# OPENAIRINTERFACE/openairinterface5g

Measured on AMD Instinct MI355X. Metric: ldpc_decoder_coded_throughput, higher is better.
Workload: dtype int8

## Files before the change

### openairinterface5g_amd/csrc/ldpc_dec_fast_core.h

```cpp
#ifndef LDPC_DEC_FAST_CORE_H
#define LDPC_DEC_FAST_CORE_H
#include "ldpc_dec_core.h"

#if !defined(__HIPCC__)
struct uint2 { uint32_t x, y; };
#endif
typedef short ldpc_v2i __attribute__((ext_vector_type(2)));
typedef unsigned short ldpc_v2u __attribute__((ext_vector_type(2)));

#if defined(__HIP_DEVICE_COMPILE__)
LDPC_HD uint32_t ldpc_perm(uint32_t s0, uint32_t s1, uint32_t sel) { return __builtin_amdgcn_perm(s0, s1, sel); }
LDPC_HD uint32_t ldpc_alignbyte(uint32_t hi, uint32_t lo, uint32_t sh) { return __builtin_amdgcn_alignbyte(hi, lo, sh); }
LDPC_HD uint32_t ldpc_umulhi(uint32_t a, uint32_t b) { return __umulhi(a, b); }
#else
LDPC_HD uint32_t ldpc_perm(uint32_t s0, uint32_t s1, uint32_t sel)
{
  const uint64_t src = ((uint64_t)s0 << 32) | s1;
  uint32_t r = 0;
  for (int i = 0; i < 4; i++) {
    const uint32_t s = (sel >> (8 * i)) & 0xff;
    const uint32_t b = s <= 7 ? (uint32_t)((src >> (8 * s)) & 0xff) : (s == 0x0c ? 0u : 0xffu);
    r |= b << (8 * i);
  }
  return r;
}
LDPC_HD uint32_t ldpc_alignbyte(uint32_t hi, uint32_t lo, uint32_t sh)
{
  return (uint32_t)(((((uint64_t)hi) << 32) | lo) >> (8 * (sh & 3)));
}
LDPC_HD uint32_t ldpc_umulhi(uint32_t a, uint32_t b) { return (uint32_t)(((uint64_t)a * b) >> 32); }
#endif

LDPC_HD ldpc_v2i ldpc_as_v2i(uint32_t x) { return __builtin_bit_cast(ldpc_v2i, x); }
LDPC_HD ldpc_v2u ldpc_as_v2u(uint32_t x) { return __builtin_bit_cast(ldpc_v2u, x); }
LDPC_HD uint32_t ldpc_u2u32(ldpc_v2u x) { return __builtin_bit_cast(uint32_t, x); }
LDPC_HD ldpc_v2u ldpc_splatu(unsigned v) { return (ldpc_v2u){(unsigned short)v, (unsigned short)v}; }
LDPC_HD ldpc_v2u ldpc_pminu(ldpc_v2u a, ldpc_v2u b) { return __builtin_elementwise_min(a, b); }
LDPC_HD ldpc_v2u ldpc_pmaxu(ldpc_v2u a, ldpc_v2u b) { return __builtin_elementwise_max(a, b); }
#define LDPC_KEY_NEUTRAL 0xfbffu
LDPC_HD ldpc_v2u ldpc_pmin3_keys(ldpc_v2u a, ldpc_v2u b, ldpc_v2u c)
{
#if defined(__HIP_DEVICE_COMPILE__)
  uint32_t r;
  asm("v_pk_maximum3_f16 %0, %1, %2, %3" : "=v"(r) : "v"(__builtin_bit_cast(uint32_t, a)), "v"(__builtin_bit_cast(uint32_t, b)),
      "v"(__builtin_bit_cast(uint32_t, c)));
  return __builtin_bit_cast(ldpc_v2u, r);
#else
  return __builtin_elementwise_min(__builtin_elementwise_min(a, b), c);
#endif
}
LDPC_HD uint32_t ldpc_as_u32(ldpc_v2i x) { return __builtin_bit_cast(uint32_t, x); }
LDPC_HD ldpc_v2i ldpc_splat(int v) { return (ldpc_v2i){(short)v, (short)v}; }
LDPC_HD ldpc_v2i ldpc_pmin(ldpc_v2i a, ldpc_v2i b) { return __builtin_elementwise_min(a, b); }
LDPC_HD ldpc_v2i ldpc_pmax(ldpc_v2i a, ldpc_v2i b) { return __builtin_elementwise_max(a, b); }
LDPC_HD ldpc_v2i ldpc_unpack_lo(uint32_t w) { return ldpc_as_v2i(ldpc_perm(0u, w, 0x0c010c00u)); }
LDPC_HD ldpc_v2i ldpc_unpack_hi(uint32_t w) { return ldpc_as_v2i(ldpc_perm(0u, w, 0x0c030c02u)); }
LDPC_HD uint32_t ldpc_pack4(ldpc_v2i lo, ldpc_v2i hi) { return ldpc_perm(ldpc_as_u32(hi), ldpc_as_u32(lo), 0x06040200u); }

struct ldpc_fast_lds {
  uint8_t *base;
  uint8_t *r;
  uint8_t *app;
  uint8_t *ext;
  const uint32_t *etbl, *ctbl, *rowtbl, *coltbl;
  const uint8_t *gllr;
  int ext_global;
};

#if defined(__HIP_DEVICE_COMPILE__)
LDPC_HD uint32_t ldpc_lds_addr(const uint8_t *p) { return (uint32_t)(uintptr_t)(const __attribute__((address_space(3))) uint8_t *)p; }
LDPC_HD uint32_t ldpc_lds_ld32(const uint8_t *, uint32_t a) { return *(const __attribute__((address_space(3))) uint32_t *)a; }
#else
LDPC_HD uint32_t ldpc_lds_addr(const uint8_t *) { return 0u; }
LDPC_HD uint32_t ldpc_lds_ld32(const uint8_t *base, uint32_t a) { return *reinterpret_cast<const uint32_t *>(base + a); }
#endif
LDPC_HD uint32_t ldpc_window_al(const uint8_t *base, uint32_t a, uint32_t sh)
{
  return ldpc_alignbyte(ldpc_lds_ld32(base, a + 4u), ldpc_lds_ld32(base, a), sh);
}
LDPC_HD uint32_t ldpc_window(const uint8_t *base, uint32_t off) { return ldpc_window_al(base, off & ~3u, off); }

LDPC_HD uint32_t ldpc_fast_odd_lanes(uint32_t parw, bool ext, uint32_t extl, uint32_t exth, int D)
{
  uint32_t np = parw >> 7;
  if (ext)
    np ^= ldpc_perm(exth, extl, 0x07050301u);
  if (D & 1)
    np = ~np;
  return np & 0x01010101u;
}
LDPC_HD uint32_t ldpc_fast_valid_lanes(int valid) { return valid > 0 ? 0x01010101u : 0u; }

template <bool IS_EXT, bool P1 = false>
LDPC_HD void ldpc_fast_cn_edge(const ldpc_fast_lds &L, uint32_t info, int t, uint32_t rw, bool first, uint32_t &dl, uint32_t &dh,
                               uint32_t &parw, uint32_t &extl, uint32_t &exth)
{
  uint32_t al, ah, rl, rh;
  if (IS_EXT) {
    const uint32_t lw = L.ext_global ? (*reinterpret_cast<const uint32_t *>(L.gllr + info + (uint32_t)t) ^ 0x80808080u)
                                     : ldpc_lds_ld32(L.base, info + (uint32_t)t);
    al = ldpc_perm(0x80808080u, lw, 0x05010400u);
    ah = ldpc_perm(0x80808080u, lw, 0x05030402u);
    if (first) {
      extl = al + (P1 ? 0x00800080u : ldpc_perm(0u, rw, 0x0c010c00u));
      exth = ah + (P1 ? 0x00800080u : ldpc_perm(0u, rw, 0x0c030c02u));
    }
    rl = 0x00800080u;
    rh = 0x00800080u;
  } else {
    const uint32_t aw = ldpc_window(L.base, info + (uint32_t)t);
    if (first)
      parw ^= aw;
    al = ldpc_perm(0x80808080u, aw, 0x05010400u);
    ah = ldpc_perm(0x80808080u, aw, 0x05030402u);
    rl = P1 ? 0x00800080u : ldpc_perm(0u, rw, 0x0c010c00u);
    rh = P1 ? 0x00800080u : ldpc_perm(0u, rw, 0x0c030c02u);
  }
  dl = al - rl;
  dh = ah - rh;
}

template <int D, bool EXT, int MODE, bool P1 = false>
LDPC_HD uint32_t ldpc_fast_cn(const ldpc_fast_lds &L, int e0, int j, int Z, int rstride, int boff_r = 0, int boff_a = 0)
{
  const int t = 4 * j + boff_r, ta = 4 * j + boff_a;
  constexpr bool KEEP = MODE == 0;
  uint32_t d_lo[MODE <= 1 ? D : 1], d_hi[MODE <= 1 ? D : 1], g_lo[KEEP ? D : 1], g_hi[KEEP ? D : 1];
  ldpc_v2u m1l = ldpc_splatu(0xffff), m2l = m1l, m1h = m1l, m2h = m1l;
  uint32_t sxl = 0, sxh = 0, parw = 0, extl = 0, exth = 0;
  uint8_t *rrow = L.r + e0 * rstride + t;
  uint8_t *rpad = rrow + (j == 0 ? Z : 0);
#pragma unroll
  for (int k = 0; k < D; k++) {
    const uint32_t info = L.etbl[e0 + k];
    const uint32_t rw = P1 ? 0u : *reinterpret_cast<const uint32_t *>(rrow + k * rstride);
    uint32_t dl, dh;
    if (EXT && k == D - 1)
      ldpc_fast_cn_edge<true, P1>(L, info, t, rw, true, dl, dh, parw, extl, exth);
    else
      ldpc_fast_cn_edge<false, P1>(L, info, ta, rw, true, dl, dh, parw, extl, exth);
    if (MODE <= 1) {
      d_lo[k] = dl;
      d_hi[k] = dh;
    }
    const ldpc_v2u ml = ldpc_pmaxu(ldpc_as_v2u(dl), ldpc_as_v2u(0x00010000u - dl));
    const ldpc_v2u mh = ldpc_pmaxu(ldpc_as_v2u(dh), ldpc_as_v2u(0x00010000u - dh));
    if (KEEP) {
      g_lo[k] = ldpc_u2u32(ml);
      g_hi[k] = ldpc_u2u32(mh);
    }
    sxl ^= dl;
    sxh ^= dh;
    m2l = ldpc_pminu(m2l, ldpc_pmaxu(m1l, ml));
    m1l = ldpc_pminu(m1l, ml);
    m2h = ldpc_pminu(m2h, ldpc_pmaxu(m1h, mh));
    m1h = ldpc_pminu(m1h, mh);
  }
  const ldpc_v2u cap = ldpc_splatu(0x8000 + 127);
  m1l = ldpc_pminu(m1l, cap); m2l = ldpc_pminu(m2l, cap);
  m1h = ldpc_pminu(m1h, cap); m2h = ldpc_pminu(m2h, cap);
  const uint32_t sl = (ldpc_u2u32(m1l) - 0x80008000u) + ldpc_u2u32(m2l), sh = (ldpc_u2u32(m1h) - 0x80008000u) + ldpc_u2u32(m2h);
  if ((D - 1) & 1) {
    sxl ^= 0x80008000u;
    sxh ^= 0x80008000u;
  }
  const uint32_t sx4 = ldpc_perm(sxh, sxl, 0x07050301u);
#pragma unroll
  for (int k = 0; k < D; k++) {
    uint32_t dl, dh;
    if (MODE <= 1) {
      dl = d_lo[k];
      dh = d_hi[k];
    } else {
      const uint32_t info = L.etbl[e0 + k];
      const uint32_t rw = P1 ? 0u : *reinterpret_cast<const uint32_t *>(rrow + k * rstride);
      if (EXT && k == D - 1)
        ldpc_fast_cn_edge<true, P1>(L, info, t, rw, false, dl, dh, parw, extl, exth);
      else
        ldpc_fast_cn_edge<false, P1>(L, info, ta, rw, false, dl, dh, parw, extl, exth);
    }
    const ldpc_v2u ml = KEEP ? ldpc_as_v2u(g_lo[k]) : ldpc_pmaxu(ldpc_as_v2u(dl), ldpc_as_v2u(0x00010000u - dl));
    const ldpc_v2u mh = KEEP ? ldpc_as_v2u(g_hi[k]) : ldpc_pmaxu(ldpc_as_v2u(dh), ldpc_as_v2u(0x00010000u - dh));
    const uint32_t ol = sl - ldpc_u2u32(ldpc_pminu(ml, m2l)), oh = sh - ldpc_u2u32(ldpc_pminu(mh, m2h));
    const uint32_t o4 = ldpc_perm(oh, ol, 0x06040200u);
    const uint32_t n4 = ((sx4 ^ ldpc_perm(dh, dl, 0x07050301u)) >> 7) & 0x01010101u;
    const uint32_t w = (o4 ^ (0x80808080u - n4)) + n4;
    *reinterpret_cast<uint32_t *>(rrow + k * rstride) = w;
    *reinterpret_cast<uint32_t *>(rpad + k * rstride) = w;
  }
  return ldpc_fast_odd_lanes(parw, EXT, extl, exth, D);
}

template <int D, bool EXT, bool P1 = false>
LDPC_HD uint32_t ldpc_fast_cn_ps(const ldpc_fast_lds &L, int e0, int j, int Z, int rstride, int boff_r = 0, int boff_a = 0)
{
  const int t = 4 * j + boff_r, ta = 4 * j + boff_a;
  constexpr int NP = D / 2;
  uint32_t m_lo[D], m_hi[D], p_lo[NP], p_hi[NP], s4[D];
  const ldpc_v2u cap = ldpc_splatu(0x8000 + 127);
  uint32_t sx4 = 0, parw = 0, extl = 0, exth = 0;
  uint8_t *rrow = L.r + e0 * rstride + t;
  uint8_t *rpad = rrow + (j == 0 ? Z : 0);
#pragma unroll
  for (int k = 0; k < D; k++) {
    const uint32_t info = L.etbl[e0 + k];
    const uint32_t rw = P1 ? 0u : *reinterpret_cast<const uint32_t *>(rrow + k * rstride);
    uint32_t dl, dh;
    if (EXT && k == D - 1)
      ldpc_fast_cn_edge<true, P1>(L, info, t, rw, true, dl, dh, parw, extl, exth);
    else
      ldpc_fast_cn_edge<false, P1>(L, info, ta, rw, true, dl, dh, parw, extl, exth);
    const ldpc_v2u ml = ldpc_pmaxu(ldpc_as_v2u(dl), ldpc_as_v2u(0x00010000u - dl));
    const ldpc_v2u mh = ldpc_pmaxu(ldpc_as_v2u(dh), ldpc_as_v2u(0x00010000u - dh));
    m_lo[k] = ldpc_u2u32(ml);
    m_hi[k] = ldpc_u2u32(mh);
    s4[k] = ldpc_perm(dh, dl, 0x07050301u);
    sx4 ^= s4[k];
    if ((k & 1) && k < D - 1) {
      const int i = k / 2;
      p_lo[i] = ldpc_u2u32(ldpc_pmin3_keys(i ? ldpc_as_v2u(p_lo[i - 1]) : cap, ldpc_as_v2u(m_lo[k - 1]), ml));
      p_hi[i] = ldpc_u2u32(ldpc_pmin3_keys(i ? ldpc_as_v2u(p_hi[i - 1]) : cap, ldpc_as_v2u(m_hi[k - 1]), mh));
    }
  }
  if (!((D - 1) & 1))
    sx4 ^= 0x80808080u;
  auto put = [&](int k, ldpc_v2u ol, ldpc_v2u oh) {
    const uint32_t o4 = ldpc_perm(ldpc_u2u32(oh), ldpc_u2u32(ol), 0x06040200u);
    const uint32_t x4 = sx4 ^ s4[k];
    const uint32_t w = (o4 ^ x4) + (x4 & 0x01010101u);
    *reinterpret_cast<uint32_t *>(rrow + k * rstride) = w;
    *reinterpret_cast<uint32_t *>(rpad + k * rstride) = w;
  };
  ldpc_v2u sl = cap, sh = cap;
  if (D & 1) {
    put(D - 1, ldpc_as_v2u(p_lo[NP - 1]), ldpc_as_v2u(p_hi[NP - 1]));
    sl = ldpc_as_v2u(m_lo[D - 1]);
    sh = ldpc_as_v2u(m_hi[D - 1]);
  }
#pragma unroll
  for (int i = NP - 1; i >= 0; i--) {
    const int k0 = 2 * i, k1 = 2 * i + 1;
    const ldpc_v2u pvl = i ? ldpc_as_v2u(p_lo[i - 1]) : cap, pvh = i ? ldpc_as_v2u(p_hi[i - 1]) : cap;
    const ldpc_v2u a0l = ldpc_as_v2u(m_lo[k0]), a0h = ldpc_as_v2u(m_hi[k0]), a1l = ldpc_as_v2u(m_lo[k1]), a1h = ldpc_as_v2u(m_hi[k1]);
    const bool last = !(D & 1) && i == NP - 1;
    put(k0, last ? ldpc_pminu(pvl, a1l) : ldpc_pmin3_keys(pvl, a1l, sl), last ? ldpc_pminu(pvh, a1h) : ldpc_pmin3_keys(pvh, a1h, sh));
    put(k1, last ? ldpc_pminu(pvl, a0l) : ldpc_pmin3_keys(pvl, a0l, sl), last ? ldpc_pminu(pvh, a0h) : ldpc_pmin3_keys(pvh, a0h, sh));
    if (i > 0) {
      sl = last ? ldpc_pminu(a0l, a1l) : ldpc_pmin3_keys(sl, a0l, a1l);
      sh = last ? ldpc_pminu(a0h, a1h) : ldpc_pmin3_keys(sh, a0h, a1h);
    }
  }
  return ldpc_fast_odd_lanes(parw, EXT, extl, exth, D);
}

template <int D, bool EXT, bool P1 = false>
LDPC_HD uint32_t ldpc_fast_cn_ps2(const ldpc_fast_lds &L, int e0a, int ja, int e0b, int jb, int Z, int rstride, uint32_t &mask_b)
{
  constexpr int N = 2, NP = D / 2;
  const int e0[N] = {e0a, e0b}, t[N] = {4 * ja, 4 * jb};
  uint32_t m_lo[N][D], m_hi[N][D], p_lo[N][NP > 0 ? NP : 1], p_hi[N][NP > 0 ? NP : 1], s4[N][D];
  const ldpc_v2u cap = ldpc_splatu(0x8000 + 127);
  uint32_t sx4[N] = {0, 0}, parw[N] = {0, 0}, extl[N] = {0, 0}, exth[N] = {0, 0};
  uint8_t *rrow[N], *rpad[N];
#pragma unroll
  for (int n = 0; n < N; n++) {
    rrow[n] = L.r + e0[n] * rstride + t[n];
    rpad[n] = rrow[n] + (t[n] == 0 ? Z : 0);
  }
#pragma unroll
  for (int k = 0; k < D; k++) {
    uint32_t info[N], rw[N];
#pragma unroll
    for (int n = 0; n < N; n++) {
      info[n] = L.etbl[e0[n] + k];
      rw[n] = P1 ? 0u : *reinterpret_cast<const uint32_t *>(rrow[n] + k * rstride);
    }
#pragma unroll
    for (int n = 0; n < N; n++) {
      uint32_t dl, dh;
      if (EXT && k == D - 1)
        ldpc_fast_cn_edge<true, P1>(L, info[n], t[n], rw[n], true, dl, dh, parw[n], extl[n], exth[n]);
      else
        ldpc_fast_cn_edge<false, P1>(L, info[n], t[n], rw[n], true, dl, dh, parw[n], extl[n], exth[n]);
      const ldpc_v2u ml = ldpc_pmaxu(ldpc_as_v2u(dl), ldpc_as_v2u(0x00010000u - dl));
      const ldpc_v2u mh = ldpc_pmaxu(ldpc_as_v2u(dh), ldpc_as_v2u(0x00010000u - dh));
      m_lo[n][k] = ldpc_u2u32(ml);
      m_hi[n][k] = ldpc_u2u32(mh);
      s4[n][k] = ldpc_perm(dh, dl, 0x07050301u);
      sx4[n] ^= s4[n][k];
      if ((k & 1) && k < D - 1) {
        const int i = k / 2;
        p_lo[n][i] = ldpc_u2u32(ldpc_pmin3_keys(i ? ldpc_as_v2u(p_lo[n][i - 1]) : cap, ldpc_as_v2u(m_lo[n][k - 1]), ml));
        p_hi[n][i] = ldpc_u2u32(ldpc_pmin3_keys(i ? ldpc_as_v2u(p_hi[n][i - 1]) : cap, ldpc_as_v2u(m_hi[n][k - 1]), mh));
      }
    }
  }
  if (!((D - 1) & 1)) {
    sx4[0] ^= 0x80808080u;
    sx4[1] ^= 0x80808080u;
  }
  auto put = [&](int n, int k, ldpc_v2u ol, ldpc_v2u oh) {
    const uint32_t o4 = ldpc_perm(ldpc_u2u32(oh), ldpc_u2u32(ol), 0x06040200u);
    const uint32_t x4 = sx4[n] ^ s4[n][k];
    const uint32_t w = (o4 ^ x4) + (x4 & 0x01010101u);
    *reinterpret_cast<uint32_t *>(rrow[n] + k * rstride) = w;
    *reinterpret_cast<uint32_t *>(rpad[n] + k * rstride) = w;
  };
  ldpc_v2u sl[N] = {cap, cap}, sh[N] = {cap, cap};
  if (D & 1) {
#pragma unroll
    for (int n = 0; n < N; n++) {
      put(n, D - 1, NP ? ldpc_as_v2u(p_lo[n][NP - 1]) : cap, NP ? ldpc_as_v2u(p_hi[n][NP - 1]) : cap);
      sl[n] = ldpc_as_v2u(m_lo[n][D - 1]);
      sh[n] = ldpc_as_v2u(m_hi[n][D - 1]);
    }
  }
#pragma unroll
  for (int i = NP - 1; i >= 0; i--) {
    const int k0 = 2 * i, k1 = 2 * i + 1;
    const bool last = !(D & 1) && i == NP - 1;
#pragma unroll
    for (int n = 0; n < N; n++) {
      const ldpc_v2u pvl = i ? ldpc_as_v2u(p_lo[n][i - 1]) : cap, pvh = i ? ldpc_as_v2u(p_hi[n][i - 1]) : cap;
      const ldpc_v2u a0l = ldpc_as_v2u(m_lo[n][k0]), a0h = ldpc_as_v2u(m_hi[n][k0]), a1l = ldpc_as_v2u(m_lo[n][k1]), a1h = ldpc_as_v2u(m_hi[n][k1]);
      put(n, k0, last ? ldpc_pminu(pvl, a1l) : ldpc_pmin3_keys(pvl, a1l, sl[n]), last ? ldpc_pminu(pvh, a1h) : ldpc_pmin3_keys(pvh, a1h, sh[n]));
      put(n, k1, last ? ldpc_pminu(pvl, a0l) : ldpc_pmin3_keys(pvl, a0l, sl[n]), last ? ldpc_pminu(pvh, a0h) : ldpc_pmin3_keys(pvh, a0h, sh[n]));
      if (i > 0) {
        sl[n] = last ? ldpc_pminu(a0l, a1l) : ldpc_pmin3_keys(sl[n], a0l, a1l);
        sh[n] = last ? ldpc_pminu(a0h, a1h) : ldpc_pmin3_keys(sh[n], a0h, a1h);
      }
    }
  }
  uint32_t out[N];
#pragma unroll
  for (int n = 0; n < N; n++) {
    out[n] = ldpc_fast_odd_lanes(parw[n], EXT, extl[n], exth[n], D);
  }
  mask_b = out[1];
  return out[0];
}
#if defined(__HIP_DEVICE_COMPILE__) && defined(LDPC_CN2_NOINLINE)
#define LDPC_CN2_ATTR __device__ __attribute__((noinline))
#else
#define LDPC_CN2_ATTR LDPC_HD
#endif
template <bool P1 = false>
LDPC_CN2_ATTR uint32_t ldpc_fast_cn2_dispatch(int deg, const ldpc_fast_lds &L, int e0a, int ja, int e0b, int jb, int Z, int rstride, uint32_t &mask_b)
{
  switch (deg) {
    case 3: return ldpc_fast_cn_ps2<3, true, P1>(L, e0a, ja, e0b, jb, Z, rstride, mask_b);
    case 4: return ldpc_fast_cn_ps2<4, true, P1>(L, e0a, ja, e0b, jb, Z, rstride, mask_b);
    default: return ldpc_fast_cn_ps2<5, true, P1>(L, e0a, ja, e0b, jb, Z, rstride, mask_b);
  }
}

#if defined(__HIP_DEVICE_COMPILE__)
__device__ __forceinline__ uint32_t ldpc_swap_pair(uint32_t v) { return (uint32_t)__builtin_amdgcn_update_dpp(0, (int)v, 0xB1 , 0xf, 0xf, false); }
template <bool P1>
__device__ __forceinline__ uint32_t ldpc_fast_cn19_pair(const ldpc_fast_lds &L, int e0, int j, int Z, int rstride, int half)
{
  constexpr int N = 10, NP = N / 2;
  const int t = 4 * j;
  const int ebase = e0 + (half ? 10 : 0);
  uint32_t m_lo[N], m_hi[N], p_lo[NP], p_hi[NP], s4[N];
  const ldpc_v2u cap = ldpc_splatu(0x8000 + 127);
  uint32_t sx4 = 0, parw = 0, extl = 0, exth = 0;
  uint8_t *rrow = L.r + ebase * rstride + t;
  uint8_t *rpad = rrow + (j == 0 ? Z : 0);
#pragma unroll
  for (int k = 0; k < N; k++) {
    const bool live = k < N - 1 || !half;
    const int kk = live ? k : N - 2;
    const uint32_t info = L.etbl[ebase + kk];
    const uint32_t rw = P1 ? 0u : *reinterpret_cast<const uint32_t *>(rrow + kk * rstride);
    uint32_t dl, dh, pw = 0;
    ldpc_fast_cn_edge<false, P1>(L, info, t, rw, true, dl, dh, pw, extl, exth);
    ldpc_v2u ml = ldpc_pmaxu(ldpc_as_v2u(dl), ldpc_as_v2u(0x00010000u - dl));
    ldpc_v2u mh = ldpc_pmaxu(ldpc_as_v2u(dh), ldpc_as_v2u(0x00010000u - dh));
    uint32_t sg = ldpc_perm(dh, dl, 0x07050301u);
    if (!live) {
      ml = mh = ldpc_splatu(LDPC_KEY_NEUTRAL);
      sg = 0u;
      pw = 0u;
    }
    m_lo[k] = ldpc_u2u32(ml); m_hi[k] = ldpc_u2u32(mh);
    s4[k] = sg;
    sx4 ^= sg;
    parw ^= pw;
    if (k & 1) {
      const int i = k / 2;
      p_lo[i] = ldpc_u2u32(ldpc_pmin3_keys(i ? ldpc_as_v2u(p_lo[i - 1]) : cap, ldpc_as_v2u(m_lo[k - 1]), ml));
      p_hi[i] = ldpc_u2u32(ldpc_pmin3_keys(i ? ldpc_as_v2u(p_hi[i - 1]) : cap, ldpc_as_v2u(m_hi[k - 1]), mh));
    }
  }
  ldpc_v2u sl = ldpc_as_v2u(ldpc_swap_pair(p_lo[NP - 1])), sh = ldpc_as_v2u(ldpc_swap_pair(p_hi[NP - 1]));
  sx4 ^= ldpc_swap_pair(sx4);
  parw ^= ldpc_swap_pair(parw);
  sx4 ^= 0x80808080u;
#pragma unroll
  for (int i = NP - 1; i >= 0; i--) {
    const ldpc_v2u pvl = i ? ldpc_as_v2u(p_lo[i - 1]) : cap, pvh = i ? ldpc_as_v2u(p_hi[i - 1]) : cap;
#pragma unroll
    for (int q = 0; q < 2; q++) {
      const int k = 2 * i + q, ko = 2 * i + 1 - q;
      const bool live = k < N - 1 || !half;
      const ldpc_v2u ol = ldpc_pmin3_keys(pvl, ldpc_as_v2u(m_lo[ko]), sl), oh = ldpc_pmin3_keys(pvh, ldpc_as_v2u(m_hi[ko]), sh);
      const uint32_t o4 = ldpc_perm(ldpc_u2u32(oh), ldpc_u2u32(ol), 0x06040200u);
      const uint32_t x4 = sx4 ^ s4[k];
      const uint32_t w = (o4 ^ x4) + (x4 & 0x01010101u);
      if (live) {
        *reinterpret_cast<uint32_t *>(rrow + k * rstride) = w;
        *reinterpret_cast<uint32_t *>(rpad + k * rstride) = w;
      }
    }
    if (i > 0) {
      sl = ldpc_pmin3_keys(sl, ldpc_as_v2u(m_lo[2 * i]), ldpc_as_v2u(m_lo[2 * i + 1]));
      sh = ldpc_pmin3_keys(sh, ldpc_as_v2u(m_hi[2 * i]), ldpc_as_v2u(m_hi[2 * i + 1]));
    }
  }
  return ldpc_fast_odd_lanes(parw, false, 0u, 0u, 19);
}
#endif

LDPC_HD uint32_t ldpc_fast_pc(const ldpc_fast_lds &L, int D, int ext, int e0, int j, int rstride)
{
  const int t = 4 * j;
  uint32_t parw = 0;
  const int ncore_edges = ext ? D - 1 : D;
  int k = 0;
  for (; k + 4 <= ncore_edges; k += 4) {
    uint32_t info[4], lo[4], hi[4];
#pragma unroll
    for (int i = 0; i < 4; i++)
      info[i] = L.etbl[e0 + k + i] + (uint32_t)t;
#pragma unroll
    for (int i = 0; i < 4; i++) {
      lo[i] = ldpc_lds_ld32(L.base, info[i] & ~3u);
      hi[i] = ldpc_lds_ld32(L.base, (info[i] & ~3u) + 4u);
    }
#pragma unroll
    for (int i = 0; i < 4; i++)
      parw ^= ldpc_alignbyte(hi[i], lo[i], info[i]);
  }
  for (; k < ncore_edges; k++)
    parw ^= ldpc_window(L.base, L.etbl[e0 + k] + (uint32_t)t);
  uint32_t extl = 0, exth = 0;
  if (ext) {
    const uint32_t info = L.etbl[e0 + D - 1];
    const uint32_t lw = L.ext_global ? (*reinterpret_cast<const uint32_t *>(L.gllr + info + (uint32_t)t) ^ 0x80808080u)
                                     : ldpc_lds_ld32(L.base, info + (uint32_t)t);
    const uint32_t rw = *reinterpret_cast<const uint32_t *>(L.r + (e0 + D - 1) * rstride + t);
    extl = ldpc_perm(0x80808080u, lw, 0x05010400u) + ldpc_perm(0u, rw, 0x0c010c00u);
    exth = ldpc_perm(0x80808080u, lw, 0x05030402u) + ldpc_perm(0u, rw, 0x0c030c02u);
  }
  return ldpc_fast_odd_lanes(parw, ext != 0, extl, exth, D);
}

#ifndef LDPC_F_MODE_D19
#define LDPC_F_MODE_D19 2
#endif
template <bool P1 = false>
LDPC_HD uint32_t ldpc_fast_cn_dispatch(int deg, int ext, const ldpc_fast_lds &L, int e0, int j, int Z, int rstride, int boff_r = 0,
                                       int boff_a = 0)
{
  if (!ext) {
    switch (deg) {
      case 19: return ldpc_fast_cn<19, false, LDPC_F_MODE_D19, P1>(L, e0, j, Z, rstride, boff_r, boff_a);
      case 10: return ldpc_fast_cn_ps<10, false, P1>(L, e0, j, Z, rstride, boff_r, boff_a);
      default: return ldpc_fast_cn_ps<8, false, P1>(L, e0, j, Z, rstride, boff_r, boff_a);
    }
  }
  switch (deg) {
    case 3: return ldpc_fast_cn_ps<3, true, P1>(L, e0, j, Z, rstride, boff_r, boff_a);
    case 4: return ldpc_fast_cn_ps<4, true, P1>(L, e0, j, Z, rstride, boff_r, boff_a);
    case 5: return ldpc_fast_cn_ps<5, true, P1>(L, e0, j, Z, rstride, boff_r, boff_a);
    case 6: return ldpc_fast_cn_ps<6, true, P1>(L, e0, j, Z, rstride, boff_r, boff_a);
    case 7: return ldpc_fast_cn_ps<7, true, P1>(L, e0, j, Z, rstride, boff_r, boff_a);
    case 8: return ldpc_fast_cn_ps<8, true, P1>(L, e0, j, Z, rstride, boff_r, boff_a);
    case 9: return ldpc_fast_cn_ps<9, true, P1>(L, e0, j, Z, rstride, boff_r, boff_a);
    default: return ldpc_fast_cn_ps<10, true, P1>(L, e0, j, Z, rstride, boff_r, boff_a);
  }
}

LDPC_HD void ldpc_fast_bn_gather_from(const ldpc_fast_lds &L, int first, int maxdeg, int j, int Z, int boff_r, uint32_t &acc_e,
                                      uint32_t &acc_o)
{
  const int u = 4 * j;
  const uint2 *tbl = reinterpret_cast<const uint2 *>(L.ctbl) + first;
  int k = 0;
  uint2 ce[4];
  if (maxdeg >= 4) {
#pragma unroll
    for (int i = 0; i < 4; i++)
      ce[i] = tbl[i];
  }
  for (; k + 4 <= maxdeg; k += 4) {
    uint32_t lo[4], hi[4], ph[4];
#pragma unroll
    for (int i = 0; i < 4; i++) {
      const uint32_t q = (uint32_t)u + ce[i].x;
      const uint32_t p = q < q - (uint32_t)Z ? q : q - (uint32_t)Z;
      const uint32_t a = ce[i].y + p + (uint32_t)boff_r;
      lo[i] = ldpc_lds_ld32(L.base, a);
      hi[i] = ldpc_lds_ld32(L.base, a + 4u);
      ph[i] = q;
    }
    if (k + 8 <= maxdeg) {
#pragma unroll
      for (int i = 0; i < 4; i++)
        ce[i] = tbl[k + 4 + i];
    }
#pragma unroll
    for (int i = 0; i < 4; i++) {
      const uint32_t w = ldpc_alignbyte(hi[i], lo[i], ph[i]);
      acc_e += w & 0x00ff00ffu;
      acc_o += (w >> 8) & 0x00ff00ffu;
    }
  }
  for (; k < maxdeg; k++) {
    const uint2 c1 = tbl[k];
    const uint32_t q = (uint32_t)u + c1.x;
    const uint32_t p = q < q - (uint32_t)Z ? q : q - (uint32_t)Z;
    const uint32_t v = ldpc_window_al(L.base, c1.y + p + (uint32_t)boff_r, q);
    acc_e += v & 0x00ff00ffu;
    acc_o += (v >> 8) & 0x00ff00ffu;
  }
}
LDPC_HD void ldpc_fast_bn_gather(const ldpc_fast_lds &L, uint32_t colrec, int maxdeg, int j, int Z, int boff_r, uint32_t &acc_e,
                                 uint32_t &acc_o)
{
  ldpc_fast_bn_gather_from(L, (int)(colrec >> 16), maxdeg, j, Z, boff_r, acc_e, acc_o);
}
LDPC_HD void ldpc_fast_bn_finish(const ldpc_fast_lds &L, int c, int deg, int j, int Z, int astride, uint32_t llr_word, uint32_t acc_e,
                                 uint32_t acc_o, int boff_a)
{
  const int u = 4 * j;
  const uint32_t lw = llr_word ^ 0x80808080u;
  acc_e += lw & 0x00ff00ffu;
  acc_o += (lw >> 8) & 0x00ff00ffu;
#if defined(__HIP_DEVICE_COMPILE__) && !defined(LDPC_NO_SAT_PK)
  const ldpc_v2i bias = ldpc_splat(deg * 128);
  uint32_t se, so;
  asm("v_sat_pk_u8_i16 %0, %1" : "=v"(se) : "v"(ldpc_as_u32(ldpc_as_v2i(acc_e) - bias)));
  asm("v_sat_pk_u8_i16 %0, %1" : "=v"(so) : "v"(ldpc_as_u32(ldpc_as_v2i(acc_o) - bias)));
  const uint32_t w = ldpc_perm(so, se, 0x05010400u);
#else
  const ldpc_v2i bias = ldpc_splat((deg + 1) * 128), lo = ldpc_splat(-128), hi = ldpc_splat(127), b128 = ldpc_splat(128);
  const ldpc_v2i ve = ldpc_pmin(ldpc_pmax(ldpc_as_v2i(acc_e) - bias, lo), hi) + b128;
  const ldpc_v2i vo = ldpc_pmin(ldpc_pmax(ldpc_as_v2i(acc_o) - bias, lo), hi) + b128;
  const uint32_t w = ldpc_perm(ldpc_as_u32(vo), ldpc_as_u32(ve), 0x06020400u);
#endif
  uint32_t *dst = reinterpret_cast<uint32_t *>(L.app + c * astride + u + boff_a);
  dst[0] = w;
  *reinterpret_cast<uint32_t *>(L.app + c * astride + u + boff_a + Z) = w;
}
LDPC_HD void ldpc_fast_bn(const ldpc_fast_lds &L, uint32_t colrec, int maxdeg, int j, int Z, int astride,
                          uint32_t llr_word, int boff_r = 0, int boff_a = 0)
{
  uint32_t acc_e = 0, acc_o = 0;
  ldpc_fast_bn_gather(L, colrec, maxdeg, j, Z, boff_r, acc_e, acc_o);
  ldpc_fast_bn_finish(L, (int)(colrec & 0xffu), (int)((colrec >> 8) & 0xffu), j, Z, astride, llr_word, acc_e, acc_o, boff_a);
}

template <int G>
LDPC_HD void ldpc_fast_bn_multi(const ldpc_fast_lds &L, const uint32_t (&rec)[G], const int (&jj)[G], const uint32_t (&lw)[G],
                                const bool (&live)[G], int md, int Z, int astride)
{
  uint32_t ae[G], at[G];
  const uint2 *tbl[G];
#pragma unroll
  for (int g = 0; g < G; g++) {
    ae[g] = at[g] = 0u;
    tbl[g] = reinterpret_cast<const uint2 *>(L.ctbl) + (int)(rec[g] >> 16);
  }
  for (int k = 0; k < md; k++) {
    uint2 ce[G];
    uint32_t lo[G], hi[G], ph[G];
#pragma unroll
    for (int g = 0; g < G; g++)
      ce[g] = tbl[g][k];
#pragma unroll
    for (int g = 0; g < G; g++) {
      const uint32_t q = 4u * (uint32_t)jj[g] + ce[g].x;
      const uint32_t p = q < q - (uint32_t)Z ? q : q - (uint32_t)Z;
      const uint32_t a = ce[g].y + p;
      lo[g] = ldpc_lds_ld32(L.base, a);
      hi[g] = ldpc_lds_ld32(L.base, a + 4u);
      ph[g] = q;
    }
#pragma unroll
    for (int g = 0; g < G; g++) {
      const uint32_t w = ldpc_alignbyte(hi[g], lo[g], ph[g]);
      ae[g] += w & 0x00ff00ffu;
      at[g] += w >> 8;
    }
  }
#pragma unroll
  for (int g = 0; g < G; g++)
    if (live[g])
      ldpc_fast_bn_finish(L, (int)(rec[g] & 0xffu), (int)((rec[g] >> 8) & 0xffu), jj[g], Z, astride, lw[g], ae[g],
                          at[g] - ((ae[g] >> 16) << 8), 0);
}

LDPC_HD int ldpc_fast_hd(const ldpc_fast_lds &L, int b, int Z, uint32_t zmagic, int astride)
{
  const int c = (int)ldpc_umulhi((uint32_t)b, zmagic), u = b - c * Z;
  return L.app[c * astride + u] < 128;
}
#endif
```

Baseline: 73.13.

## Compute check-node differences in sign-magnitude via packed f16 subtract and even/odd unpack

Replaces the offset-binary unpack, integer subtract and max(d, -d) magnitude computation with a packed half-precision subtract that yields sign-magnitude words directly. The magnitude key becomes a single OR, and sign bits are gathered with the perm sign-replicate selectors. Bytes are unpacked into even and odd lanes with a cheap AND plus one perm, and the output repack selector is changed to match. This cuts per-edge VALU instructions in the check-node update. It relies on the f16 bit patterns of small offset integers behaving like sign-magnitude, and the host emulation is extended to mirror this.

```diff
diff --git a/openairinterface5g_amd/csrc/ldpc_dec_fast_core.h b/openairinterface5g_amd/csrc/ldpc_dec_fast_core.h
--- a/openairinterface5g_amd/csrc/ldpc_dec_fast_core.h
+++ b/openairinterface5g_amd/csrc/ldpc_dec_fast_core.h
@@ -19,7 +19,9 @@
   uint32_t r = 0;
   for (int i = 0; i < 4; i++) {
     const uint32_t s = (sel >> (8 * i)) & 0xff;
-    const uint32_t b = s <= 7 ? (uint32_t)((src >> (8 * s)) & 0xff) : (s == 0x0c ? 0u : 0xffu);
+    const uint32_t b = s <= 7    ? (uint32_t)((src >> (8 * s)) & 0xff)
+                       : s <= 11 ? (((src >> (16 * (s - 8) + 15)) & 1) ? 0xffu : 0u)
+                                 : (s == 0x0c ? 0u : 0xffu);
     r |= b << (8 * i);
   }
   return r;
@@ -49,6 +51,24 @@
   return __builtin_elementwise_min(__builtin_elementwise_min(a, b), c);
 #endif
 }
+LDPC_HD uint32_t ldpc_psub_sm(uint32_t a, uint32_t r)
+{
+#if defined(__HIP_DEVICE_COMPILE__)
+  typedef _Float16 ldpc_v2h __attribute__((ext_vector_type(2)));
+  const uint32_t d = __builtin_bit_cast(uint32_t, __builtin_bit_cast(ldpc_v2h, a) - __builtin_bit_cast(ldpc_v2h, r));
+  return d;
+#else
+  uint32_t d = 0;
+  for (int h = 0; h < 32; h += 16) {
+    const uint32_t x = (a >> h) & 0xffffu, y = (r >> h) & 0xffffu;
+    d |= (x < y ? 0x8000u | (y - x) : x - y) << h;
+  }
+  return d;
+#endif
+}
+LDPC_HD ldpc_v2u ldpc_sm_key(uint32_t d) { return __builtin_bit_cast(ldpc_v2u, d | 0x80008000u); }
+LDPC_HD uint32_t ldpc_unpack_even(uint32_t w) { return w & 0x00ff00ffu; }
+LDPC_HD uint32_t ldpc_unpack_odd(uint32_t w) { return ldpc_perm(0u, w, 0x0c030c01u); }
 LDPC_HD uint32_t ldpc_as_u32(ldpc_v2i x) { return __builtin_bit_cast(uint32_t, x); }
 LDPC_HD ldpc_v2i ldpc_splat(int v) { return (ldpc_v2i){(short)v, (short)v}; }
 LDPC_HD ldpc_v2i ldpc_pmin(ldpc_v2i a, ldpc_v2i b) { return __builtin_elementwise_min(a, b); }
@@ -80,11 +100,14 @@
 }
 LDPC_HD uint32_t ldpc_window(const uint8_t *base, uint32_t off) { return ldpc_window_al(base, off & ~3u, off); }
 
+#define LDPC_SEL_EO 0x07030501u
+#define LDPC_SEL_SIGNS 0x0b090a08u
+template <uint32_t SEL = 0x07050301u>
 LDPC_HD uint32_t ldpc_fast_odd_lanes(uint32_t parw, bool ext, uint32_t extl, uint32_t exth, int D)
 {
   uint32_t np = parw >> 7;
   if (ext)
-    np ^= ldpc_perm(exth, extl, 0x07050301u);
+    np ^= ldpc_perm(exth, extl, SEL);
   if (D & 1)
     np = ~np;
   return np & 0x01010101u;
@@ -92,32 +115,31 @@
 LDPC_HD uint32_t ldpc_fast_valid_lanes(int valid) { return valid > 0 ? 0x01010101u : 0u; }
 
 template <bool IS_EXT, bool P1 = false>
-LDPC_HD void ldpc_fast_cn_edge(const ldpc_fast_lds &L, uint32_t info, int t, uint32_t rw, bool first, uint32_t &dl, uint32_t &dh,
-                               uint32_t &parw, uint32_t &extl, uint32_t &exth)
-{
-  uint32_t al, ah, rl, rh;
+LDPC_HD void ldpc_fast_cn_edge(const ldpc_fast_lds &L, uint32_t info, int t, uint32_t rw, bool first, uint32_t &de, uint32_t &dod,
+                               uint32_t &parw, uint32_t &exte, uint32_t &exto)
+{
   if (IS_EXT) {
     const uint32_t lw = L.ext_global ? (*reinterpret_cast<const uint32_t *>(L.gllr + info + (uint32_t)t) ^ 0x80808080u)
                                      : ldpc_lds_ld32(L.base, info + (uint32_t)t);
-    al = ldpc_perm(0x80808080u, lw, 0x05010400u);
-    ah = ldpc_perm(0x80808080u, lw, 0x05030402u);
+    const uint32_t ae = ldpc_unpack_even(lw), ao = ldpc_unpack_odd(lw);
     if (first) {
-      extl = al + (P1 ? 0x00800080u : ldpc_perm(0u, rw, 0x0c010c00u));
-      exth = ah + (P1 ? 0x00800080u : ldpc_perm(0u, rw, 0x0c030c02u));
-    }
-    rl = 0x00800080u;
-    rh = 0x00800080u;
+      exte = ae + (P1 ? 0x00800080u : ldpc_unpack_even(rw));
+      exto = ao + (P1 ? 0x00800080u : ldpc_unpack_odd(rw));
+    }
+    de = ldpc_psub_sm(ae, 0x00800080u);
+    dod = ldpc_psub_sm(ao, 0x00800080u);
   } else {
     const uint32_t aw = ldpc_window(L.base, info + (uint32_t)t);
     if (first)
       parw ^= aw;
-    al = ldpc_perm(0x80808080u, aw, 0x05010400u);
-    ah = ldpc_perm(0x80808080u, aw, 0x05030402u);
-    rl = P1 ? 0x00800080u : ldpc_perm(0u, rw, 0x0c010c00u);
-    rh = P1 ? 0x00800080u : ldpc_perm(0u, rw, 0x0c030c02u);
-  }
-  dl = al - rl;
-  dh = ah - rh;
+    if (P1) {
+      de = ldpc_psub_sm(ldpc_unpack_even(aw), 0x00800080u);
+      dod = ldpc_psub_sm(ldpc_unpack_odd(aw), 0x00800080u);
+    } else {
+      de = ldpc_psub_sm(ldpc_unpack_even(aw), ldpc_unpack_even(rw));
+      dod = ldpc_psub_sm(ldpc_unpack_odd(aw), ldpc_unpack_odd(rw));
+    }
+  }
 }
 
 template <int D, bool EXT, int MODE, bool P1 = false>
@@ -143,8 +165,8 @@
       d_lo[k] = dl;
       d_hi[k] = dh;
     }
-    const ldpc_v2u ml = ldpc_pmaxu(ldpc_as_v2u(dl), ldpc_as_v2u(0x00010000u - dl));
-    const ldpc_v2u mh = ldpc_pmaxu(ldpc_as_v2u(dh), ldpc_as_v2u(0x00010000u - dh));
+    const ldpc_v2u ml = ldpc_sm_key(dl);
+    const ldpc_v2u mh = ldpc_sm_key(dh);
     if (KEEP) {
       g_lo[k] = ldpc_u2u32(ml);
       g_hi[k] = ldpc_u2u32(mh);
@@ -160,11 +182,7 @@
   m1l = ldpc_pminu(m1l, cap); m2l = ldpc_pminu(m2l, cap);
   m1h = ldpc_pminu(m1h, cap); m2h = ldpc_pminu(m2h, cap);
   const uint32_t sl = (ldpc_u2u32(m1l) - 0x80008000u) + ldpc_u2u32(m2l), sh = (ldpc_u2u32(m1h) - 0x80008000u) + ldpc_u2u32(m2h);
-  if ((D - 1) & 1) {
-    sxl ^= 0x80008000u;
-    sxh ^= 0x80008000u;
-  }
-  const uint32_t sx4 = ldpc_perm(sxh, sxl, 0x07050301u);
+  const uint32_t sx4 = ldpc_perm(sxh, sxl, LDPC_SEL_EO);
 #pragma unroll
   for (int k = 0; k < D; k++) {
     uint32_t dl, dh;
@@ -179,16 +197,16 @@
       else
         ldpc_fast_cn_edge<false, P1>(L, info, ta, rw, false, dl, dh, parw, extl, exth);
     }
-    const ldpc_v2u ml = KEEP ? ldpc_as_v2u(g_lo[k]) : ldpc_pmaxu(ldpc_as_v2u(dl), ldpc_as_v2u(0x00010000u - dl));
-    const ldpc_v2u mh = KEEP ? ldpc_as_v2u(g_hi[k]) : ldpc_pmaxu(ldpc_as_v2u(dh), ldpc_as_v2u(0x00010000u - dh));
+    const ldpc_v2u ml = KEEP ? ldpc_as_v2u(g_lo[k]) : ldpc_sm_key(dl);
+    const ldpc_v2u mh = KEEP ? ldpc_as_v2u(g_hi[k]) : ldpc_sm_key(dh);
     const uint32_t ol = sl - ldpc_u2u32(ldpc_pminu(ml, m2l)), oh = sh - ldpc_u2u32(ldpc_pminu(mh, m2h));
-    const uint32_t o4 = ldpc_perm(oh, ol, 0x06040200u);
-    const uint32_t n4 = ((sx4 ^ ldpc_perm(dh, dl, 0x07050301u)) >> 7) & 0x01010101u;
+    const uint32_t o4 = ldpc_perm(oh, ol, 0x06020400u);
+    const uint32_t n4 = ((sx4 ^ ldpc_perm(dh, dl, LDPC_SEL_EO)) >> 7) & 0x01010101u;
     const uint32_t w = (o4 ^ (0x80808080u - n4)) + n4;
     *reinterpret_cast<uint32_t *>(rrow + k * rstride) = w;
     *reinterpret_cast<uint32_t *>(rpad + k * rstride) = w;
   }
-  return ldpc_fast_odd_lanes(parw, EXT, extl, exth, D);
+  return ldpc_fast_odd_lanes<LDPC_SEL_EO>(parw, EXT, extl, exth, D);
 }
 
 template <int D, bool EXT, bool P1 = false>
@@ -210,11 +228,11 @@
       ldpc_fast_cn_edge<true, P1>(L, info, t, rw, true, dl, dh, parw, extl, exth);
     else
       ldpc_fast_cn_edge<false, P1>(L, info, ta, rw, true, dl, dh, parw, extl, exth);
-    const ldpc_v2u ml = ldpc_pmaxu(ldpc_as_v2u(dl), ldpc_as_v2u(0x00010000u - dl));
-    const ldpc_v2u mh = ldpc_pmaxu(ldpc_as_v2u(dh), ldpc_as_v2u(0x00010000u - dh));
+    const ldpc_v2u ml = ldpc_sm_key(dl);
+    const ldpc_v2u mh = ldpc_sm_key(dh);
     m_lo[k] = ldpc_u2u32(ml);
     m_hi[k] = ldpc_u2u32(mh);
-    s4[k] = ldpc_perm(dh, dl, 0x07050301u);
+    s4[k] = ldpc_perm(dh, dl, LDPC_SEL_SIGNS);
     sx4 ^= s4[k];
     if ((k & 1) && k < D - 1) {
       const int i = k / 2;
@@ -222,10 +240,9 @@
       p_hi[i] = ldpc_u2u32(ldpc_pmin3_keys(i ? ldpc_as_v2u(p_hi[i - 1]) : cap, ldpc_as_v2u(m_hi[k - 1]), mh));
     }
   }
-  if (!((D - 1) & 1))
-    sx4 ^= 0x80808080u;
+  sx4 ^= 0x80808080u;
   auto put = [&](int k, ldpc_v2u ol, ldpc_v2u oh) {
-    const uint32_t o4 = ldpc_perm(ldpc_u2u32(oh), ldpc_u2u32(ol), 0x06040200u);
+    const uint32_t o4 = ldpc_perm(ldpc_u2u32(oh), ldpc_u2u32(ol), 0x06020400u);
     const uint32_t x4 = sx4 ^ s4[k];
     const uint32_t w = (o4 ^ x4) + (x4 & 0x01010101u);
     *reinterpret_cast<uint32_t *>(rrow + k * rstride) = w;
@@ -250,7 +267,7 @@
       sh = last ? ldpc_pminu(a0h, a1h) : ldpc_pmin3_keys(sh, a0h, a1h);
     }
   }
-  return ldpc_fast_odd_lanes(parw, EXT, extl, exth, D);
+  return ldpc_fast_odd_lanes<LDPC_SEL_EO>(parw, EXT, extl, exth, D);
 }
 
 template <int D, bool EXT, bool P1 = false>
@@ -282,11 +299,11 @@
         ldpc_fast_cn_edge<true, P1>(L, info[n], t[n], rw[n], true, dl, dh, parw[n], extl[n], exth[n]);
       else
         ldpc_fast_cn_edge<false, P1>(L, info[n], t[n], rw[n], true, dl, dh, parw[n], extl[n], exth[n]);
-      const ldpc_v2u ml = ldpc_pmaxu(ldpc_as_v2u(dl), ldpc_as_v2u(0x00010000u - dl));
-      const ldpc_v2u mh = ldpc_pmaxu(ldpc_as_v2u(dh), ldpc_as_v2u(0x00010000u - dh));
+      const ldpc_v2u ml = ldpc_sm_key(dl);
+      const ldpc_v2u mh = ldpc_sm_key(dh);
       m_lo[n][k] = ldpc_u2u32(ml);
       m_hi[n][k] = ldpc_u2u32(mh);
-      s4[n][k] = ldpc_perm(dh, dl, 0x07050301u);
+      s4[n][k] = ldpc_perm(dh, dl, LDPC_SEL_SIGNS);
       sx4[n] ^= s4[n][k];
       if ((k & 1) && k < D - 1) {
         const int i = k / 2;
@@ -295,12 +312,10 @@
       }
     }
   }
-  if (!((D - 1) & 1)) {
-    sx4[0] ^= 0x80808080u;
-    sx4[1] ^= 0x80808080u;
-  }
+  sx4[0] ^= 0x80808080u;
+  sx4[1] ^= 0x80808080u;
   auto put = [&](int n, int k, ldpc_v2u ol, ldpc_v2u oh) {
-    const uint32_t o4 = ldpc_perm(ldpc_u2u32(oh), ldpc_u2u32(ol), 0x06040200u);
+    const uint32_t o4 = ldpc_perm(ldpc_u2u32(oh), ldpc_u2u32(ol), 0x06020400u);
     const uint32_t x4 = sx4[n] ^ s4[n][k];
     const uint32_t w = (o4 ^ x4) + (x4 & 0x01010101u);
     *reinterpret_cast<uint32_t *>(rrow[n] + k * rstride) = w;
@@ -334,7 +349,7 @@
   uint32_t out[N];
 #pragma unroll
   for (int n = 0; n < N; n++) {
-    out[n] = ldpc_fast_odd_lanes(parw[n], EXT, extl[n], exth[n], D);
+    out[n] = ldpc_fast_odd_lanes<LDPC_SEL_EO>(parw[n], EXT, extl[n], exth[n], D);
   }
   mask_b = out[1];
   return out[0];
@@ -375,9 +390,9 @@
     const uint32_t rw = P1 ? 0u : *reinterpret_cast<const uint32_t *>(rrow + kk * rstride);
     uint32_t dl, dh, pw = 0;
     ldpc_fast_cn_edge<false, P1>(L, info, t, rw, true, dl, dh, pw, extl, exth);
-    ldpc_v2u ml = ldpc_pmaxu(ldpc_as_v2u(dl), ldpc_as_v2u(0x00010000u - dl));
-    ldpc_v2u mh = ldpc_pmaxu(ldpc_as_v2u(dh), ldpc_as_v2u(0x00010000u - dh));
-    uint32_t sg = ldpc_perm(dh, dl, 0x07050301u);
+    ldpc_v2u ml = ldpc_sm_key(dl);
+    ldpc_v2u mh = ldpc_sm_key(dh);
+    uint32_t sg = ldpc_perm(dh, dl, LDPC_SEL_SIGNS);
     if (!live) {
       ml = mh = ldpc_splatu(LDPC_KEY_NEUTRAL);
       sg = 0u;
@@ -405,7 +420,7 @@
       const int k = 2 * i + q, ko = 2 * i + 1 - q;
       const bool live = k < N - 1 || !half;
       const ldpc_v2u ol = ldpc_pmin3_keys(pvl, ldpc_as_v2u(m_lo[ko]), sl), oh = ldpc_pmin3_keys(pvh, ldpc_as_v2u(m_hi[ko]), sh);
-      const uint32_t o4 = ldpc_perm(ldpc_u2u32(oh), ldpc_u2u32(ol), 0x06040200u);
+      const uint32_t o4 = ldpc_perm(ldpc_u2u32(oh), ldpc_u2u32(ol), 0x06020400u);
       const uint32_t x4 = sx4 ^ s4[k];
       const uint32_t w = (o4 ^ x4) + (x4 & 0x01010101u);
       if (live) {
```

Result: faster. 75.93, median of 6 (+3.8%).
